# Jackxiini/Tensorflow-distributed-learning

Measured on AMD Instinct MI355X. Metric: images/sec (whole node) MNIST CNN global_batch=64*N, higher is better.
Workload: dtype fp32; 1 GPU; global_batch=64, parallelism=dp1, engine=fused, communicator=local, variant=reference, process_model=single, communicator_impl=LocalCommunicator, ipc_mode=dmabuf, allreduce=local, steps_per_execution=25, graph_captured=True, input_prefetch_executions=1, allreduce_in_graph=False, replicas_identical=True

## Files before the change

csrc/kernels/mnist_cnn.hip:

```cpp
#include <type_traits>

#include "common.h"
#include "mnist_cnn.h"
#include "optim.h"
#include "xgmi_device.h"

namespace tdl {

struct HeadWeights {
  float wa[10], wb[10], b4[10], b3a, b3b;
};

__device__ __forceinline__ HeadWeights load_head_weights(const MnistArgs& a, int l) {
  HeadWeights hw;
  const float* w4 = a.W + a.ow4;
#pragma unroll
  for (int c = 0; c < 10; ++c) {
    hw.wa[c] = w4[l * 10 + c];
    hw.wb[c] = w4[(l + 64) * 10 + c];
    hw.b4[c] = a.W[a.ob4 + c];
  }
  hw.b3a = a.W[a.ob3 + l];
  hw.b3b = a.W[a.ob3 + l + 64];
  return hw;
// ... 426 lines not shown
      const unsigned q = qdc[j];
      const unsigned s = (unsigned)sel[j];
      const f4 v = vdc[j];
      st4(dCs + e4 * 4, f4{(q & 0xffu) == s ? v.x : 0.f, ((q >> 8) & 0xffu) == s ? v.y : 0.f,
                           ((q >> 16) & 0xffu) == s ? v.z : 0.f, (q >> 24) == s ? v.w : 0.f});
    }
  }
#pragma unroll
  for (int j = 0; j < kIp1; ++j) {
    const int e4 = tid + j * 512;
    if (e4 < 169 * 8) st4(P1s + (e4 >> 3) * kP1StrideB + (e4 & 7) * 4, vp1[j]);
  }
#pragma unroll
  for (int j = 0; j < kIwd; ++j) {
    const int e4 = tid + j * 512;
    if (e4 < kLdsWd / 4) st4(Wd + e4 * 4, vwd[j]);
  }
  if (tid < 196) st4(Xs + tid * 4, vx);
  stamp(a.stamps, 1);
  __syncthreads();
  stamp(a.stamps, 2);

  {
    const int t0 = kWgradTiles[half][wave][0], ntiles = kWgradTiles[half][wave][1];
    for (int j = 0; j < ntiles; ++j) {
      const int mt = t0 + j;
      const bool bias_tile = mt == 18;
      const int k = mt * 16 + i;
      const int tap = bias_tile ? 0 : k >> 5, ci = k & 31;
      const int kh = tap / 3, kw = tap - kh * 3;
      const float* pa0 = P1s + (kh * 13 + kw + g) * kP1StrideB + ci;
      const float* paS = pa0 + (g >= 2 ? 3 * kP1StrideB : 0);
      const float* pb0 = dCs + (2 * kDcDim + 2 + g) * kDcStride + 16 * p + i;
      const float* pbS = pb0 + (g >= 2 ? 5 * kDcStride : 0);
      const float unit_a = (i == 0) ? 1.f : 0.f;
      auto kloop = [&](auto bias) {
        f4 c0 = zero4(), c1 = zero4();
#pragma unroll
        for (int s0 = 0; s0 < 25; s0 += 5) {
          float av[5], bv[5];
#pragma unroll
          for (int u = 0; u < 5; ++u) {
            const int st = s0 + u, q = (4 * st) / 10, r = (4 * st) % 10;
            const bool strad = r == 8;
            if constexpr (decltype(bias)::value) av[u] = unit_a;
            else av[u] = (strad ? paS : pa0)[(q * 13 + r) * kP1StrideB];
            bv[u] = (strad ? pbS : pb0)[(q * kDcDim + r) * kDcStride];
          }
#pragma unroll
          for (int u = 0; u < 5; ++u) {
            if ((s0 + u) & 1) c1 = mfma16x16x4(av[u], bv[u], c1);
            else c0 = mfma16x16x4(av[u], bv[u], c0);
          }
        }
        return c0 + c1;
      };
      const f4 acc = bias_tile ? kloop(std::true_type{}) : kloop(std::false_type{});
#pragma unroll
      for (int r = 0; r < 4; ++r) {
        const int row = mt * 16 + 4 * g + r;
        if (row < kMnistPart2Rows) a.part2[((size_t)bi * kMnistPart2Rows + row) * 64 + 16 * p + i] = acc[r];
      }
    }
  }

  stamp(a.stamps, 3);
  float dw[10];
#pragma unroll
  for (int j = 0; j < 10; ++j) dw[j] = 0.f;
  const int d = 7 - wave;
  const int pix0 = half ? kDgSplit : 0, pix1 = half ? 169 : kDgSplit;
  if (d < (pix1 - pix0 + 15) / 16) {
    const int P = pix0 + d * 16 + i;
    const bool valid = P < pix1;
    const int Pc = valid ? P : pix0;
    const int ih = Pc / 13, iw = Pc - ih * 13;
    const float* wb = Wd + (g * 16 + i) * 4;
    const int c = 16 * h + i;
    unsigned q1v[4];
#pragma unroll
    for (int r = 0; r < 4; ++r) {
      const int Pr = min(pix0 + d * 16 + 4 * g + r, pix1 - 1);
      q1v[r] = a.A1[((size_t)bi * 169 + Pr) * 32 + c];
    }
    const int ih_lo = (pix0 + d * 16) / 13, ih_hi = min(pix0 + d * 16 + 15, pix1 - 1) / 13;
    const int kh_lo = max(0, ih_lo - 9), kh_hi = min(2, ih_hi);
    f4 acc0 = zero4(), acc1 = zero4();
    for (int kh = kh_lo; kh <= kh_hi; ++kh) {
#pragma unroll
      for (int kw = 0; kw < 3; ++kw) {
        const int tap = kh * 3 + kw;
        const float* ap = dCs + ((ih - kh + 2) * kDcDim + (iw - kw + 2)) * kDcStride + 4 * g;
#pragma unroll
        for (int c0 = 0; c0 < 64; c0 += 16) {
          const f4 av = ld4(ap + c0);
          const f4 bv = ld4(wb + (tap * 16 + c0 / 4) * 64);
          acc0 = mfma16x16x4(av.x, bv.x, acc0);
          acc1 = mfma16x16x4(av.y, bv.y, acc1);
          acc0 = mfma16x16x4(av.z, bv.z, acc0);
          acc1 = mfma16x16x4(av.w, bv.w, acc1);
        }
      }
    }
    const f4 acc = acc0 + acc1;
    stamp(a.stamps, 6);
#pragma unroll
    for (int r = 0; r < 4; ++r) {
      const int Pr = pix0 + d * 16 + 4 * g + r;
      if (Pr < pix1) {
        const float v = P1s[Pr * kP1StrideB + c] > 0.f ? acc[r] : 0.f;
        const unsigned q1 = q1v[r];
        const int ph = Pr / 13, pw = Pr - ph * 13;
        const float* img = Xs + (2 * ph + (q1 >> 1)) * 28 + 2 * pw + (q1 & 1);
#pragma unroll
        for (int kh = 0; kh < 3; ++kh)
#pragma unroll
          for (int kw = 0; kw < 3; ++kw) dw[kh * 3 + kw] = fmaf(img[kh * 28 + kw], v, dw[kh * 3 + kw]);
        dw[9] += v;
      }
    }
  }
#pragma unroll
  for (int j = 0; j < 10; ++j) dw[j] = sum_lane_groups(dw[j]);
  if (g == 0) {
#pragma unroll
    for (int j = 0; j < 10; ++j) red[(wave * 10 + j) * 16 + i] = dw[j];
  }
  stamp(a.stamps, 4);
  __syncthreads();
  stamp(a.stamps, 5);
  if (tid < 160) {
    const int j = tid >> 4, ii = tid & 15;
    float s = 0.f;
#pragma unroll
    for (int w = 2; w < 8; ++w) s += red[(w * 10 + j) * 16 + ii];
    a.part1[((size_t)bi * 2 + half) * kMnistPart1Cols + j * 32 + 16 * h + ii] = s;
  }
}

constexpr int kLdsFwd = 784 + 320 + 169 * kP1Stride + 72 * 16 * 4 + 400 + 169 * 32 / 4 + 400 / 4 + 16 * 128 + 4 + 128 +
                        288 * 16 +
                        kHeadW;
constexpr int kDcF = 15, kDcFStride = 20;
constexpr int kLdsFwdFused = kLdsFwd + kDcF * kDcF * kDcFStride;
constexpr int kP1Live = 12;
constexpr int kConv1Tiles = kP1Live * kP1Live / 4;
__constant__ int kFusedWgradTiles[8][2] = {{0, 2}, {3, 2}, {7, 3}, {12, 3}, {2, 1}, {5, 2}, {10, 2}, {15, 3}};

__device__ __forceinline__ void bwd_stamp(unsigned long long* buf, int k) {
  if (buf != nullptr && (threadIdx.x & 63) == 0)
    buf[(size_t)gridDim.x * 72 + (blockIdx.x * 8 + (threadIdx.x >> 6)) * 4 + k] = __builtin_amdgcn_s_memrealtime();
}

template <int N>
__device__ __forceinline__ void fused_wgrad_tiles(const MnistArgs& a, int bi, int cq, int t0, const float* P1s,
                                                  const float* dCs) {
  const int lane = threadIdx.x & 63, i = lane & 15, g = lane >> 4;
  const float* pa0[N];
#pragma unroll
  for (int u = 0; u < N; ++u) {
    const int k = (t0 + u) * 16 + i;
    const int tap = k >> 5, ci = k & 31;
    const int kh = tap / 3, kw = tap - kh * 3;
    pa0[u] = P1s + (kh * 13 + kw + g) * kP1Stride + ci;
  }
  const int wrapA = g >= 2 ? 3 * kP1Stride : 0, wrapB = g >= 2 ? 5 * kDcFStride : 0;
  const float* pb0 = dCs + (2 * kDcF + 2 + g) * kDcFStride + i;
  f4 acc[N];
#pragma unroll
  for (int u = 0; u < N; ++u) acc[u] = zero4();
  constexpr int kS = 3, kBlocks = (25 + kS - 1) / kS;
  float bv[2][kS], av[2][kS][N];
  auto load = [&](int buf, int blk) {
#pragma unroll
    for (int j = 0; j < kS; ++j) {
      const int st = blk * kS + j;
      if (st >= 25) break;
      const int q = (4 * st) / 10, r = (4 * st) % 10;
      const bool strad = r == 8;
      bv[buf][j] = pb0[(q * kDcF + r) * kDcFStride + (strad ? wrapB : 0)];
#pragma unroll
      for (int u = 0; u < N; ++u) av[buf][j][u] = pa0[u][(q * 13 + r) * kP1Stride + (strad ? wrapA : 0)];
    }
  };
  load(0, 0);
#pragma unroll
  for (int blk = 0; blk < kBlocks; ++blk) {
    if (blk + 1 < kBlocks) load((blk + 1) & 1, blk + 1);
    __builtin_amdgcn_sched_barrier(0);
#pragma unroll
    for (int j = 0; j < kS; ++j) {
      if (blk * kS + j >= 25) break;
#pragma unroll
      for (int u = 0; u < N; ++u) acc[u] = mfma16x16x4(av[blk & 1][j][u], bv[blk & 1][j], acc[u]);
    }
    __builtin_amdgcn_sched_barrier(0);
  }
  const auto rs = buf_rsrc(a.part2 + (size_t)bi * kP2QuadFloats, kP2QuadFloats * 4);
#pragma unroll
  for (int u = 0; u < N; ++u) st4_sc1(rs, ((((t0 + u) * 4 + g) * 64 + 16 * cq + i) * 4) * 4, acc[u]);
}

__device__ __forceinline__ void lds_dgrad_w2(const float* w2d, f4 (&bwd)[9]) {
  const int wave = __builtin_amdgcn_readfirstlane(threadIdx.x >> 6), lane = threadIdx.x & 63;
  const int i = lane & 15, g = lane >> 4, nt = wave >> 2;
#pragma unroll
  for (int tap = 0; tap < 9; ++tap) bwd[tap] = ld4(w2d + (tap * 32 + 16 * nt + i) * 16 + 4 * g);
}

__device__ __forceinline__ void fused_conv_bwd(const MnistArgs& a, int bi, int cq, const float* dp2s,
                                               const uint8_t* a2s, const float* P1s, const uint8_t* a1s,
                                               const float* xs, float* dCs, float* red, const f4 (&bwd)[9]) {
  const int tid = threadIdx.x, wave = __builtin_amdgcn_readfirstlane(tid >> 6), lane = tid & 63;
  const int i = lane & 15, g = lane >> 4;
  bwd_stamp(a.stamps, 0);

  auto wgrad = [&]() {
    const int t0 = kFusedWgradTiles[wave][0], ntiles = kFusedWgradTiles[wave][1];
    if (ntiles == 2) fused_wgrad_tiles<2>(a, bi, cq, t0, P1s, dCs);
    else if (ntiles == 3) fused_wgrad_tiles<3>(a, bi, cq, t0, P1s, dCs);
    else fused_wgrad_tiles<1>(a, bi, cq, t0, P1s, dCs);
  };
  const bool swap = (a.variant & kMnistVariantStagger) && wave >= 4;
  if (!swap) wgrad();
  bwd_stamp(a.stamps, 1);

  float dw[10];
#pragma unroll
  for (int j = 0; j < 10; ++j) dw[j] = 0.f;
  const int nt = wave >> 2, wt = wave & 3;
  auto dgrad = [&](auto ktiles) {
    constexpr int kT = decltype(ktiles)::value;
    const int ci = 16 * nt + i;
    f4 acc[kT][2];
    int ih[kT], iw[kT], khlo[kT], khhi[kT];
#pragma unroll
    for (int u = 0; u < kT; ++u) {
      const int t = wt + 4 * u;
      const int Pc = min(t * 16 + i, 168);
      ih[u] = Pc / 13;
      iw[u] = Pc - ih[u] * 13;
      const int ih_lo = min(t * 16, 168) / 13, ih_hi = min(t * 16 + 15, 168) / 13;
      khlo[u] = t < 11 ? max(0, ih_lo - 9) : 3;
      khhi[u] = min(2, ih_hi);
      acc[u][0] = zero4();
      acc[u][1] = zero4();
    }
    float p1v[kT][4];
    unsigned q1v[kT][4];
#pragma unroll
    for (int u = 0; u < kT; ++u)
#pragma unroll
      for (int r = 0; r < 4; ++r) {
        const int Pr = min((wt + 4 * u) * 16 + 4 * g + r, 168);
        p1v[u][r] = P1s[Pr * kP1Stride + ci];
        q1v[u][r] = a1s[Pr * 32 + ci];
      }
    f4 av[2][kT];
    auto load = [&](int buf, int tap) {
      const int kh = tap / 3, kw = tap - kh * 3;
#pragma unroll
      for (int u = 0; u < kT; ++u)
        av[buf][u] = ld4(dCs + ((ih[u] - kh + 2) * kDcF + (iw[u] - kw + 2)) * kDcFStride + 4 * g);
    };
    load(0, 0);
#pragma unroll
    for (int tap = 0; tap < 9; ++tap) {
      if (tap + 1 < 9) load((tap + 1) & 1, tap + 1);
      __builtin_amdgcn_sched_barrier(0);
      const int kh = tap / 3;
      const f4 bv = bwd[tap];
#pragma unroll
      for (int u = 0; u < kT; ++u) {
        if (kh < khlo[u] || kh > khhi[u]) continue;
        const f4 x = av[tap & 1][u];
        acc[u][0] = mfma16x16x4(x.x, bv.x, acc[u][0]);
        acc[u][1] = mfma16x16x4(x.y, bv.y, acc[u][1]);
        acc[u][0] = mfma16x16x4(x.z, bv.z, acc[u][0]);
        acc[u][1] = mfma16x16x4(x.w, bv.w, acc[u][1]);
      }
      __builtin_amdgcn_sched_barrier(0);
    }
#pragma unroll
    for (int u = 0; u < kT; ++u) {
      const int t = wt + 4 * u;
      if (t >= 11) continue;
      const f4 ac = acc[u][0] + acc[u][1];
#pragma unroll
      for (int r = 0; r < 4; ++r) {
        const int Pr = t * 16 + 4 * g + r;
        if (Pr < 169) {
          const float v = p1v[u][r] > 0.f ? ac[r] : 0.f;
          const unsigned q1 = q1v[u][r];
          const int ph = Pr / 13, pw = Pr - ph * 13;
          const float* img = xs + (2 * ph + (q1 >> 1)) * 28 + 2 * pw + (q1 & 1);
#pragma unroll
          for (int kh = 0; kh < 3; ++kh)
#pragma unroll
            for (int kw = 0; kw < 3; ++kw) dw[kh * 3 + kw] = fmaf(img[kh * 28 + kw], v, dw[kh * 3 + kw]);
          dw[9] += v;
        }
      }
    }
  };
  if (wt < 2) dgrad(std::integral_constant<int, 3>{});
  else dgrad(std::integral_constant<int, 2>{});
  if (swap) wgrad();
  bwd_stamp(a.stamps, 2);
#pragma unroll
  for (int j = 0; j < 10; ++j) dw[j] = sum_lane_groups(dw[j]);
  if (g == 0) {
#pragma unroll
    for (int j = 0; j < 10; ++j) red[(wave * 10 + j) * 16 + i] = dw[j];
  }
  lds_barrier();
  bwd_stamp(a.stamps, 3);
  if (tid < kMnistPart1Cols) {
    const int j = tid >> 5, c = tid & 31, nt = c >> 4, ii = c & 15;
    float sum = 0.f;
#pragma unroll
    for (int w = 0; w < 4; ++w) sum += red[((4 * nt + w) * 10 + j) * 16 + ii];
    a.part1[((size_t)bi * 4 + cq) * kMnistPart1Cols + tid] = sum;
  }
}

__device__ __forceinline__ void store_saved_fwd(const MnistArgs& a, int bi, int cq, const float* P1s,
                                                const uint8_t* a1s, const float* p2s, const uint8_t* a2s,
                                                int t, int nt) {
  for (int e = (a.fused_bwd ? 676 : 0) + t; e < (a.fused_bwd ? 776 : 2 * 338 + 200); e += nt) {
    if (e < 338) {
      const int e4 = cq * 338 + e, pos = e4 >> 3, c4 = (e4 & 7) * 4;
      st4(a.P1 + (size_t)bi * 5408 + e4 * 4, ld4(P1s + pos * kP1Stride + c4));
    } else if (e < 676) {
      const int w = cq * 338 + (e - 338);
      reinterpret_cast<unsigned*>(a.A1 + (size_t)bi * 5408)[w] = reinterpret_cast<const unsigned*>(a1s)[w];
    } else if (e < 776) {
      const int u = e - 676, wo = u >> 2, q = u & 3;
      st4(a.P2 + (size_t)bi * 1600 + wo * 64 + 16 * cq + 4 * q, ld4(p2s + wo * 16 + 4 * q));
    } else {
      const int u = e - 776, wo = u >> 2, q = u & 3;
      *reinterpret_cast<unsigned*>(a.A2 + (size_t)bi * 1600 + wo * 64 + 16 * cq + 4 * q) =
          reinterpret_cast<const unsigned*>(a2s)[wo * 4 + q];
    }
  }
}

__global__ __launch_bounds__(512) void k_fwd_conv(MnistArgs a) {
  extern __shared__ __attribute__((aligned(16))) float sm[];
  float* xs = sm;
  float* w1s = xs + 784;
  float* P1s = w1s + 320;
  float* w2s = P1s + 169 * kP1Stride;
  float* p2s = w2s + 72 * 16 * 4;
  uint8_t* a1s = reinterpret_cast<uint8_t*>(p2s + 400);
  uint8_t* a2s = a1s + 169 * 32;
  float* red = reinterpret_cast<float*>(a2s + 400);
  int* s_last = reinterpret_cast<int*>(red + 16 * 128);
  float* w2d = red + 16 * 128 + 4 + 128;
  float* hws = w2d + 288 * 16;
  float* dCs = hws + kHeadW;
  const int tid = threadIdx.x, wave = tid >> 6, lane = tid & 63;
  const int i = lane & 15, g = lane >> 4;
  int bi = blockIdx.x >> 2, cq = blockIdx.x & 3;
  if ((a.variant & kMnistVariantXcd) && (a.b & 7) == 0) {
    const int x = blockIdx.x & 7, sl = blockIdx.x >> 3;
    bi = x * (a.b >> 3) + (sl >> 2);
    cq = sl & 3;
  }
  if ((a.variant & kMnistVariantPrio) && __builtin_amdgcn_readfirstlane(wave) >= 4) __builtin_amdgcn_s_setprio(1);
  stamp(a.stamps, 0);
  const int sample = a.idx[bi];
  const f4 vx = ld4(a.X + (size_t)sample * 784 + min(tid, 195) * 4);
  const int label = a.Y[sample];
  const float vw1 = tid < 288 ? a.W[a.ow1 + tid] : a.W[a.ob1 + min(tid - 288, 31)];
  f4 vw2[3];
#pragma unroll
  for (int j = 0; j < 3; ++j) {
    const int e = min(tid + j * 512, 1151);
    vw2[j] = ld4(a.W + a.ow2 + (e >> 2) * 64 + 16 * cq + (e & 3) * 4);
  }
  const float b2v = a.W[a.ob2 + 16 * cq + (lane & 15)];
  const uint32_t tag = a.ep[0] + 1u;
  __builtin_amdgcn_sched_barrier(0);
  if (tid < 196) st4(xs + tid * 4, vx);
  if (tid < 320) w1s[tid] = vw1;
#pragma unroll
  for (int j = 0; j < 3; ++j) {
    const int e = tid + j * 512;
    if (e < 1152) {
      const int k = e >> 2, q = e & 3;
      float* d = w2s + ((k >> 2) * 16 + 4 * q) * 4 + (k & 3);
      d[0] = vw2[j].x;
      d[4] = vw2[j].y;
      d[8] = vw2[j].z;
      d[12] = vw2[j].w;
      st4(w2d + k * 16 + 4 * q, vw2[j]);
    }
  }
  stamp(a.stamps, 1);
  __syncthreads();
  stamp(a.stamps, 2);
  const int n4 = (tid & 31) * 4, rg = tid >> 5;
  f4 w3v[25];
  const auto w3r = buf_rsrc(a.W + a.ow3 + (size_t)16 * cq * 128, (unsigned)((1600 - 16 * cq) * 128 * 4));
  const int w3vo = (rg * 128 + n4) * 4;
  auto ldw3 = [&](int j) { w3v[j] = ld4_buf(w3r, w3vo, j * 64 * 128 * 4); };
#pragma unroll
  for (int j = 0; j < 6; ++j) ldw3(j);
  {
    float bw[2][3];
#pragma unroll
    for (int nt = 0; nt < 2; ++nt)
#pragma unroll
      for (int s3 = 0; s3 < 3; ++s3) {
        const int k = 4 * s3 + g;
        bw[nt][s3] = k < 9 ? w1s[k * 32 + nt * 16 + i] : 0.f;
      }
    int tap_off[3];
#pragma unroll
    for (int s3 = 0; s3 < 3; ++s3) {
      const int k = min(4 * s3 + g, 8);
      tap_off[s3] = (k / 3) * 28 + (k % 3);
    }
    const float bias[2] = {w1s[288 + i], w1s[288 + 16 + i]};
    const int cwave = __builtin_amdgcn_readfirstlane(wave);
    static_assert(kConv1Tiles == 4 * 6 + 4 * 3, "slot -> tile map of conv1");
    auto live = [&](int it, int u) { return cwave < 4 || 2 * it + u < 3; };
    const int mtb = wave < 4 ? wave : 20 + wave;
    float xa[2][2][3];
    auto load_x = [&](int buf, int it) {
      const int mt0 = mtb + 8 * it;
#pragma unroll
      for (int u = 0; u < 2; ++u) {
        if (!live(it, u)) continue;
        const int w = (mt0 + 4 * u) * 4 + (i >> 2), q = i & 3;
        const int ph = w / kP1Live;
        const int y = 2 * ph + (q >> 1), x = 2 * (w - ph * kP1Live) + (q & 1);
        const float* xb = xs + y * 28 + x;
#pragma unroll
        for (int s3 = 0; s3 < 3; ++s3) xa[buf][u][s3] = xb[tap_off[s3]];
      }
    };
    load_x(0, 0);
#pragma unroll
    for (int it = 0; it < 3; ++it) {
      const int mt0 = mtb + 8 * it;
      f4 acc[2][2];
#pragma unroll
      for (int u = 0; u < 2; ++u)
#pragma unroll
        for (int nt = 0; nt < 2; ++nt) acc[u][nt] = zero4();
#pragma unroll
      for (int s3 = 0; s3 < 3; ++s3)
#pragma unroll
        for (int u = 0; u < 2; ++u) {
          if (!live(it, u)) continue;
#pragma unroll
          for (int nt = 0; nt < 2; ++nt) acc[u][nt] = mfma16x16x4(xa[it & 1][u][s3], bw[nt][s3], acc[u][nt]);
        }
// ... 4 lines not shown
#pragma unroll
        for (int j = 6 + 5 * it; j < 11 + 5 * it; ++j) ldw3(j);
        __builtin_amdgcn_sched_barrier(0);
      }
#pragma unroll
      for (int u = 0; u < 2; ++u) {
        if (!live(it, u)) continue;
        const int w = (mt0 + 4 * u) * 4 + g;
        const int ph = w / kP1Live;
        const int wo = ph * 13 + (w - ph * kP1Live);
#pragma unroll
        for (int nt = 0; nt < 2; ++nt) {
          const f4 ac = acc[u][nt];
          float m = ac.x;
          unsigned am = 0;
          if (ac.y > m) { m = ac.y; am = 1; }
          if (ac.z > m) { m = ac.z; am = 2; }
          if (ac.w > m) { m = ac.w; am = 3; }
          const int co = nt * 16 + i;
          const float v = fmaxf(m + bias[nt], 0.f);
          P1s[wo * kP1Stride + co] = v;
          a1s[wo * 32 + co] = (uint8_t)am;
        }
      }
    }
    if (cwave >= 4) {
      const int e = tid - 256;
      if (e < 25 * 8) {
        const int c = e >> 3, c4 = e & 7;
        const int cell = c < 13 ? 12 * 13 + c : (c - 13) * 13 + 12;
        st4(P1s + cell * kP1Stride + 4 * c4, zero4());
        reinterpret_cast<unsigned*>(a1s)[cell * 8 + c4] = 0u;
      }
    }
  }
  stamp(a.stamps, 3);
  lds_barrier();
  stamp(a.stamps, 4);
  if (wave < 7) {
    const int wi = wave * 4 + (i >> 2), q = i & 3;
    const bool valid = wi < 25;
    const int wic = valid ? wi : 0;
    const int ph = wic / 5, pw = wic - ph * 5;
    const int oh = 2 * ph + (q >> 1), ow = 2 * pw + (q & 1);
    const float* ab = P1s + (oh * 13 + ow) * kP1Stride + 4 * g;
    const float* bb = w2s + (g * 16 + i) * 4;
    f4 acc0 = zero4(), acc1 = zero4();
#pragma unroll
    for (int kk = 0; kk < 9; ++kk) {
      const int kh = kk / 3, kw = kk % 3;
#pragma unroll
      for (int cb = 0; cb < 32; cb += 16) {
        const f4 av = ld4(ab + (kh * 13 + kw) * kP1Stride + cb);
        const f4 bv = ld4(bb + ((kk * 32 + cb) / 4) * 64);
        acc0 = mfma16x16x4(av.x, bv.x, acc0);
        acc1 = mfma16x16x4(av.y, bv.y, acc1);
        acc0 = mfma16x16x4(av.z, bv.z, acc0);
        acc1 = mfma16x16x4(av.w, bv.w, acc1);
      }
      __builtin_amdgcn_sched_barrier(0);
      ldw3(16 + kk);
      __builtin_amdgcn_sched_barrier(0);
    }
    const f4 acc = acc0 + acc1;
    stamp(a.stamps, 5);
    const int wo = wave * 4 + g;
    if (wo < 25) {
      float m = acc.x;
      unsigned am = 0;
      if (acc.y > m) { m = acc.y; am = 1; }
      if (acc.z > m) { m = acc.z; am = 2; }
      if (acc.w > m) { m = acc.w; am = 3; }
      const float v = fmaxf(m + b2v, 0.f);
      p2s[wo * 16 + i] = v;
      a2s[wo * 16 + i] = (uint8_t)am;
    }
  } else {
#pragma unroll
    for (int j = 16; j < 25; ++j) ldw3(j);
    if (a.head != 0) {
      float hv[23];
#pragma unroll
      for (int u = 0; u < 23; ++u) {
        const int e = min(lane + 64 * u, 1417);
        hv[u] = a.W[e < 1280 ? a.ow4 + e : (e < 1408 ? a.ob3 + (e - 1280) : a.ob4 + (e - 1408))];
      }
#pragma unroll
      for (int u = 0; u < 23; ++u)
        if (lane + 64 * u < 1418) hws[lane + 64 * u] = hv[u];
    }
    if (a.head == 1 && a.dp2_fwd && a.fused_bwd) {
      for (int e4 = lane; e4 < kDcF * kDcF * kDcFStride / 4; e4 += 64) st4(dCs + e4 * 4, zero4());
    }
  }
  __syncthreads();
  {
    f4 hs = zero4();
#pragma unroll
    for (int j = 0; j < 25; ++j) hs += p2s[j * 16 + rg] * w3v[j];
    st4(red + rg * 128 + n4, hs);
  }
  lds_barrier();
  const bool tagged = a.head == 1 && a.dp2_fwd;
  float* sown = red + 16 * 128 + 4;
  if (tid < 32) {
    f4 hsum = zero4();
#pragma unroll
    for (int k = 0; k < 16; ++k) hsum += ld4(red + k * 128 + 4 * tid);
    if (!tagged) {
      st4_sc1(buf_rsrc(a.part3 + ((size_t)cq * a.b + bi) * 128, 512), tid * 16, hsum);
    } else {
      st4(sown + 4 * tid, hsum);
      unsigned long long* p = a.part3t + ((size_t)cq * a.b + bi) * 128 + 4 * tid;
      const unsigned long long tg = (unsigned long long)tag << 32;
      __hip_atomic_store(p, (unsigned long long)__float_as_uint(hsum.x) | tg, __ATOMIC_RELAXED, __HIP_MEMORY_SCOPE_AGENT);
      __hip_atomic_store(p + 1, (unsigned long long)__float_as_uint(hsum.y) | tg, __ATOMIC_RELAXED,
                         __HIP_MEMORY_SCOPE_AGENT);
      __hip_atomic_store(p + 2, (unsigned long long)__float_as_uint(hsum.z) | tg, __ATOMIC_RELAXED,
                         __HIP_MEMORY_SCOPE_AGENT);
      __hip_atomic_store(p + 3, (unsigned long long)__float_as_uint(hsum.w) | tg, __ATOMIC_RELAXED,
                         __HIP_MEMORY_SCOPE_AGENT);
    }
  }
  stamp(a.stamps, 6);
  if (a.head == 0) {
    store_saved_fwd(a, bi, cq, P1s, a1s, p2s, a2s, tid, 512);
    return;
  }
  HeadWeights hw;
  const int uwave = __builtin_amdgcn_readfirstlane(wave);
  if (uwave == 0) hw = lds_head_weights(hws, lane);
  f4 bwd[9];
  if (a.head == 1 && a.dp2_fwd && a.fused_bwd) lds_dgrad_w2(w2d, bwd);

  if (!tagged) {
    asm volatile("s_waitcnt vmcnt(0)" ::: "memory");
    __syncthreads();
    if (tid == 0) {
      const unsigned old = __hip_atomic_fetch_add(a.cnt + bi, 1u, __ATOMIC_RELAXED, __HIP_MEMORY_SCOPE_AGENT);
      s_last[0] = (old & 3u) == 3u;
    }
  }
  lds_barrier();
  const bool last = tagged || s_last[0] != 0;
  float* sdh = red;
  if (last && uwave == 0) {
    if (a.head == 1) head_row(a, bi, lane, label, hw, sdh, tag, tagged ? sown : nullptr, cq, !tagged || cq == kHeadQuarter);
    else head_eval(a, bi, lane, label, hw);
  }
  if (a.head != 1) return;
  if (!last) store_saved_fwd(a, bi, cq, P1s, a1s, p2s, a2s, tid, 512);
  else if (wave != 0) store_saved_fwd(a, bi, cq, P1s, a1s, p2s, a2s, tid - 64, 448);
  if (!a.dp2_fwd) return;
  lds_barrier();
  if (a.fused_bwd) stamp(a.stamps, 7);
  const f4 dh = ld4(sdh + n4);
  float v[25];
  {
    typedef float f2 __attribute__((ext_vector_type(2)));
    const f2 dlo = {dh.x, dh.y}, dhi = {dh.z, dh.w};
#pragma unroll
    for (int j = 0; j < 25; ++j) {
      f2 t = f2{w3v[j].x, w3v[j].y} * dlo;
      t = __builtin_elementwise_fma(f2{w3v[j].z, w3v[j].w}, dhi, t);
      v[j] = t.x + t.y;
    }
  }
  const float d = reduce_scatter32<25>(v, lane);
  const int j = lane & 31;
  if (a.fused_bwd) {
    float val = 0.f;
    if (j < 25) {
      const int kk = j * 16 + rg;
      val = p2s[kk] > 0.f ? d : 0.f;
      const unsigned am = a2s[kk];
      const int ph = (j * 13) >> 6, pw = j - 5 * ph;
      const int y = 2 * ph + (int)(am >> 1), x = 2 * pw + (int)(am & 1u);
      dCs[((y + 2) * kDcF + x + 2) * kDcFStride + rg] = val;
    }
    float sb = rs_swap16(val, val);
    sb += dpp_xor8(sb);
    sb += dpp_mirror8(sb);
    sb += dpp_xor2(sb);
    sb += dpp_xor1(sb);
    if (j == 0) {
      const auto rs = buf_rsrc(a.part2 + (size_t)bi * kP2QuadFloats, kP2QuadFloats * 4);
      st4_sc1(rs, (((kP2Quads - 1) * 64 + 16 * cq + rg) * 4) * 4, f4{sb, 0.f, 0.f, 0.f});
    }
    lds_barrier();
    fused_conv_bwd(a, bi, cq, p2s, a2s, P1s, a1s, xs, dCs, red, bwd);
    return;
  }
  if (j < 25) {
    const int kk = j * 16 + rg;
    a.dP2[(size_t)bi * 1600 + j * 64 + 16 * cq + rg] = p2s[kk] > 0.f ? d : 0.f;
  }
  stamp(a.stamps, 7);
}

__global__ __launch_bounds__(256) void k_finalize(MnistArgs a, int apply_sgd, int ndb, int nbs, int nb2, int nb1) {
  const float lr = *a.lr;
  int blk = blockIdx.x;
  if (blk < ndb) {
    const int T = blk * 4 + (threadIdx.x >> 6);
    if (T < kDenseTasks) dense_w_task(a, T, threadIdx.x & 63, apply_sgd != 0, lr);
    return;
  }
  blk -= ndb;
  if (blk < nbs) {
    const int e = a.ow3 + blk * 256 + threadIdx.x;
    if (e < a.nslab) a.W[e] -= lr * a.G[e];
    return;
  }
  if (blk < nbs + nb2) {
    const int t = (blk - nbs) * 256 + threadIdx.x;
    const int o = t >> 2, sub = t & 3;
    const int n = kMnistPart2Rows * 64;
    float s = 0.f;
    const int oc = min(o, n - 1);
    const int e = (oc >> 6) < 288 ? a.ow2 + oc : a.ob2 + (oc & 63);
    const float wold = apply_sgd ? a.W[e] : 0.f;
    for (int base = 0; base < a.b; base += 64) {
      float v[16];
#pragma unroll
      for (int j = 0; j < 16; ++j) v[j] = a.part2[(size_t)min(base + sub + 4 * j, a.b - 1) * n + oc];
#pragma unroll
      for (int j = 0; j < 16; ++j) s += (base + sub + 4 * j < a.b) ? v[j] : 0.f;
    }
    s += __shfl_xor(s, 1, 64);
    s += __shfl_xor(s, 2, 64);
    if (sub == 0 && o < n) {
      a.G[e] = s;
      if (apply_sgd) a.W[e] = wold - lr * s;
    }
    return;
  }
  const int t = (blk - nbs - nb2) * 256 + threadIdx.x;
  const int o = t >> 4, sub = t & 15;
  const int rows = mnist_part1_rows(a.b, a.fused_bwd != 0);
  float s = 0.f;
  const int oc = min(o, kMnistPart1Cols - 1);
  const int e = oc < 288 ? a.ow1 + oc : a.ob1 + (oc - 288);
  const float wold = apply_sgd ? a.W[e] : 0.f;
  for (int base = 0; base < rows; base += 128) {
    float v[8];
#pragma unroll
    for (int j = 0; j < 8; ++j) v[j] = a.part1[(size_t)min(base + sub + 16 * j, rows - 1) * kMnistPart1Cols + oc];
#pragma unroll
    for (int j = 0; j < 8; ++j) s += (base + sub + 16 * j < rows) ? v[j] : 0.f;
  }
#pragma unroll
  for (int m = 1; m < 16; m <<= 1) s += __shfl_xor(s, m, 64);
  if (sub == 0 && o < kMnistPart1Cols) {
    a.G[e] = s;
    if (apply_sgd) a.W[e] = wold - lr * s;
  }
}

__device__ __forceinline__ void fx_range(const MnistArgs& a, int j, int& lo, int& cnt, int& nseg, int& stride) {
  nseg = 1;
  stride = 0;
  if (j < kFxW3) {
    lo = a.ow3 + (j >> 1) * 2048 + (j & 1) * 64;
    cnt = 64;
    nseg = 16;
    stride = 128;
  } else if (j < kFxW3 + 4) {
    lo = a.ob3 + 32 * (j - kFxW3);
    cnt = 32;
  } else if (j < kFxW3 + 8) {
    lo = a.ow4 + 320 * (j - kFxW3 - 4);
    cnt = 320;
  } else if (j == kFxW3 + 8) {
    lo = a.ob4;
    cnt = 10;
  } else if (j < kFxDense + kFxConv2) {
    const int qd = (j - kFxDense) >> 1, h = (j - kFxDense) & 1;
    if (qd == kP2Quads - 1) {
      lo = a.ob2 + 32 * h;
      cnt = 32;
    } else {
      lo = a.ow2 + qd * 256 + 32 * h;
      cnt = 32;
      nseg = 4;
      stride = 64;
    }
  } else {
    const int q = j - kFxDense - kFxConv2;
    lo = q < 18 ? a.ow1 + q * 16 : a.ob1 + (q - 18) * 16;
    cnt = 16;
  }
}

template <int R>
__device__ __forceinline__ void finalize_x_body(const MnistArgs& a, int apply_sgd, int j);

template <int R, bool LOOP>
__global__ __launch_bounds__(512) void k_finalize_x(MnistArgs a, int apply_sgd) {
  unsigned long long* sb = a.stamps == nullptr ? nullptr
      : a.stamps + (size_t)a.b * 4 * 104 + ((size_t)blockIdx.x * 8 + (threadIdx.x >> 6)) * 2;
  if (sb != nullptr && (threadIdx.x & 63) == 0) sb[0] = __builtin_amdgcn_s_memrealtime();
  if constexpr (LOOP) {
    for (int j = blockIdx.x; j < kFxBlocks; j += gridDim.x) {
      finalize_x_body<R>(a, apply_sgd, j);
      __syncthreads();
    }
  } else {
    finalize_x_body<R>(a, apply_sgd, blockIdx.x);
  }
  if (sb != nullptr && (threadIdx.x & 63) == 0) sb[1] = __builtin_amdgcn_s_memrealtime();
}

template <int R>
__device__ __forceinline__ void finalize_x_body(const MnistArgs& a, int apply_sgd, int j) {
  const int tid = threadIdx.x, wave = tid >> 6, lane = tid & 63;
  const float lr = *a.lr;
  const bool xchg = R > 1 && a.xchg && apply_sgd;
  if (j == 0 && tid == 4 * 64) a.ep[0] += 1u;
  uint32_t e = 0;
  float* xdst = nullptr;
  int64_t half = 0;
  if (xchg) {
    e = __builtin_amdgcn_readfirstlane(a.xa.epoch[j]) + 1u;
    if (xgmi_failed(a.xa.err)) {
      if (tid == 0) a.xa.epoch[j] = e;
      return;
    }
    half = (int64_t)(e & 1u) * 2 * a.xa.cap;
    xdst = a.xa.p.buf[a.xa.rank] + half;
  }
  const bool sgd_local = R == 1 && apply_sgd;
  const bool keep_g = !((sgd_local || xchg) && (a.variant & kMnistVariantNoG));
  if (j < kFxW3) {
    if (wave < 4) dense_w_task(a, (j >> 1) * 8 + (j & 1) * 4 + wave, lane, sgd_local, lr, xdst, keep_g);
  } else if (j < kFxDense) {
    const int jj = j - kFxW3, t = 2 * jj + wave;
    if (jj < 8 ? wave < 2 : wave == 0)
      dense_w_task(a, jj < 8 ? (t < 8 ? kD1TasksW3 - 8 + t : kD1TasksW3 + t - 8) : kD1TasksW3 + 8, lane, sgd_local, lr,
                   xdst, keep_g);
  } else if (j < kFxDense + kFxConv2) {
    __shared__ f4 fx_red2[8][32];
    const int qd = (j - kFxDense) >> 1, h = (j - kFxDense) & 1, c = tid & 31, grp = tid >> 5;
    const bool biasq = qd == kP2Quads - 1;
// ... 241 lines not shown
```

Measured before the change: 2.765 million images/sec.

## Software-pipeline fused conv dgrad epilogue with MFMA and hoist address precompute

Restructures the fused conv backward dgrad: each tile's ReLU-masked weight-gradient FMAs for the previous tile are interleaved with the next tile's MFMAs using sched_group_barriers. Tap counts per tile are specialised at compile time, so tiles outside the valid kernel rows do no work. Address offsets, P1 values and the first wgrad operand block are precomputed before the barrier, off the critical path. The cost is more register pressure and more complex scheduling.

```diff
diff --git a/csrc/kernels/mnist_cnn.hip b/csrc/kernels/mnist_cnn.hip
--- a/csrc/kernels/mnist_cnn.hip
+++ b/csrc/kernels/mnist_cnn.hip
@@ -602,24 +602,72 @@
     buf[(size_t)gridDim.x * 72 + (blockIdx.x * 8 + (threadIdx.x >> 6)) * 4 + k] = __builtin_amdgcn_s_memrealtime();
 }
 
+__device__ __forceinline__ void dgrad_mfma_stamp(unsigned long long* buf) {
+#ifdef TDL_DIAG_DGRAD_STAMP
+  if (buf != nullptr && (threadIdx.x & 63) == 0)
+    buf[(size_t)gridDim.x * 104 + kFxBlocks * 16 + blockIdx.x * 8 + (threadIdx.x >> 6)] = __builtin_amdgcn_s_memrealtime();
+#endif
+}
+
+constexpr int kWgS = 3;
+struct FusedBwdPre {
+  int wga[3], wgb;
+  float wav[kWgS][3];
+  int dga[3], xo[3][4];
+  float p1v[3][4];
+};
+
+__device__ __forceinline__ int wg_wrap_a(int g) { return g >= 2 ? 3 * kP1Stride : 0; }
+
+__device__ __forceinline__ void fused_bwd_pre(FusedBwdPre& pre, const float* P1s, const uint8_t* a1s) {
+  const int wave = __builtin_amdgcn_readfirstlane(threadIdx.x >> 6), lane = threadIdx.x & 63;
+  const int i = lane & 15, g = lane >> 4;
+  const int t0 = kFusedWgradTiles[wave][0];
+#pragma unroll
+  for (int u = 0; u < 3; ++u) {
+    const int k = min(t0 + u, 17) * 16 + i;
+    const int tap = k >> 5, ci = k & 31;
+    const int kh = tap / 3, kw = tap - kh * 3;
+    pre.wga[u] = (kh * 13 + kw + g) * kP1Stride + ci;
+  }
+  pre.wgb = (2 * kDcF + 2 + g) * kDcFStride + i;
+#pragma unroll
+  for (int j = 0; j < kWgS; ++j) {
+    const int q = (4 * j) / 10, r = (4 * j) % 10;
+#pragma unroll
+    for (int u = 0; u < 3; ++u) pre.wav[j][u] = P1s[pre.wga[u] + (q * 13 + r) * kP1Stride + (r == 8 ? wg_wrap_a(g) : 0)];
+  }
+  const int nt = wave >> 2, wt = wave & 3, ci = 16 * nt + i;
+#pragma unroll
+  for (int u = 0; u < 3; ++u) {
+    const int t = wt + 4 * u;
+    const int Pc = min(t * 16 + i, 168);
+    const int ih = Pc / 13, iw = Pc - ih * 13;
+    pre.dga[u] = ((ih + 2) * kDcF + iw + 2) * kDcFStride + 4 * g;
+#pragma unroll
+    for (int r = 0; r < 4; ++r) {
+      const int Pr = min(t * 16 + 4 * g + r, 168);
+      pre.p1v[u][r] = P1s[Pr * kP1Stride + ci];
+      const int q1 = a1s[Pr * 32 + ci];
+      const int ph = Pr / 13, pw = Pr - ph * 13;
+      pre.xo[u][r] = (2 * ph + (q1 >> 1)) * 28 + 2 * pw + (q1 & 1);
+    }
+  }
+}
+
 template <int N>
 __device__ __forceinline__ void fused_wgrad_tiles(const MnistArgs& a, int bi, int cq, int t0, const float* P1s,
-                                                  const float* dCs) {
+                                                  const float* dCs, const FusedBwdPre& pre) {
   const int lane = threadIdx.x & 63, i = lane & 15, g = lane >> 4;
   const float* pa0[N];
 #pragma unroll
-  for (int u = 0; u < N; ++u) {
-    const int k = (t0 + u) * 16 + i;
-    const int tap = k >> 5, ci = k & 31;
-    const int kh = tap / 3, kw = tap - kh * 3;
-    pa0[u] = P1s + (kh * 13 + kw + g) * kP1Stride + ci;
-  }
-  const int wrapA = g >= 2 ? 3 * kP1Stride : 0, wrapB = g >= 2 ? 5 * kDcFStride : 0;
-  const float* pb0 = dCs + (2 * kDcF + 2 + g) * kDcFStride + i;
+  for (int u = 0; u < N; ++u) pa0[u] = P1s + pre.wga[u];
+  const int wrapA = wg_wrap_a(g), wrapB = g >= 2 ? 5 * kDcFStride : 0;
+  const float* pb0 = dCs + pre.wgb;
   f4 acc[N];
 #pragma unroll
   for (int u = 0; u < N; ++u) acc[u] = zero4();
-  constexpr int kS = 3, kBlocks = (25 + kS - 1) / kS;
+  constexpr int kS = kWgS, kBlocks = (25 + kS - 1) / kS;
   float bv[2][kS], av[2][kS][N];
   auto load = [&](int buf, int blk) {
 #pragma unroll
@@ -630,7 +678,8 @@
       const bool strad = r == 8;
       bv[buf][j] = pb0[(q * kDcF + r) * kDcFStride + (strad ? wrapB : 0)];
 #pragma unroll
-      for (int u = 0; u < N; ++u) av[buf][j][u] = pa0[u][(q * 13 + r) * kP1Stride + (strad ? wrapA : 0)];
+      for (int u = 0; u < N; ++u)
+        av[buf][j][u] = blk == 0 ? pre.wav[j][u] : pa0[u][(q * 13 + r) * kP1Stride + (strad ? wrapA : 0)];
     }
   };
   load(0, 0);
@@ -658,18 +707,134 @@
   for (int tap = 0; tap < 9; ++tap) bwd[tap] = ld4(w2d + (tap * 32 + 16 * nt + i) * 16 + 4 * g);
 }
 
+constexpr int dg_kh_lo(int t) { return (16 * t) / 13 > 9 ? (16 * t) / 13 - 9 : 0; }
+constexpr int dg_kh_hi(int t) { return (16 * t + 15) / 13 < 2 ? (16 * t + 15) / 13 : 2; }
+constexpr int dg_taps(int t) { return 3 * (dg_kh_hi(t) - dg_kh_lo(t) + 1); }
+static_assert(dg_taps(2) == 9 && dg_taps(3) == 9 && dg_taps(6) == 9 && dg_taps(7) == 9, "tile class 2");
+static_assert(dg_taps(0) == 6 && dg_taps(4) == 9 && dg_taps(8) == 9 && dg_taps(1) == 9 && dg_taps(5) == 9 &&
+              dg_taps(9) == 3, "tile classes 0 and 1");
+
+#define TDL_SGB(mask, n) __builtin_amdgcn_sched_group_barrier(mask, n, 0)
+
+template <int WTC>
+__device__ __forceinline__ void fused_dgrad(const FusedBwdPre& pre, const float* dCs, const float* xs,
+                                            const f4 (&bwd)[9], float (&dw)[10], unsigned long long* stamps) {
+  constexpr int kT = WTC < 2 ? 3 : 2;
+  auto lda = [&](int u, int tap) {
+    const int kh = tap / 3, kw = tap - kh * 3;
+    return ld4(dCs + pre.dga[u] - (kh * kDcF + kw) * kDcFStride);
+  };
+  auto ldx = [&](int u, int k, int r) { return xs[pre.xo[u][r] + (k / 3) * 28 + k % 3]; };
+  f4 acc0 = zero4(), acc1 = zero4(), pacc0 = zero4(), pacc1 = zero4();
+  float v[4] = {0.f, 0.f, 0.f, 0.f};
+  f4 av[2];
+  float ev[2][12];
+  float el[9][4];
+  av[0] = lda(0, 3 * dg_kh_lo(WTC));
+  auto tile = [&](auto uc, auto sc) {
+    constexpr int u = decltype(uc)::value, t = WTC + 4 * u, up = u > 0 ? u - 1 : 0;
+    constexpr int s0 = decltype(sc)::value;
+    constexpr int tap0 = 3 * dg_kh_lo(t), nA = dg_taps(t);
+    constexpr int cps = u > 0 ? 9 / nA : 0;
+    constexpr int lps = u + 1 == kT ? 9 / nA : 0;
+    static_assert((u == 0 || cps * nA == 9) && (u + 1 < kT || lps * nA == 9), "epilogue split over the taps");
+    acc0 = zero4();
+    acc1 = zero4();
+#pragma unroll
+    for (int j = 0; j < nA; ++j) {
+      const int p = (s0 + j) & 1;
+      if (j + 1 < nA) {
+        av[p ^ 1] = lda(u, tap0 + j + 1);
+#pragma unroll
+        for (int e = 0; e < 4 * cps; ++e) ev[p ^ 1][e] = ldx(up, (j + 1) * cps + (e >> 2), e & 3);
+      } else if constexpr (u + 1 < kT) {
+        constexpr int ncps = 9 / dg_taps(t + 4);
+        av[p ^ 1] = lda(u + 1, 3 * dg_kh_lo(t + 4));
+#pragma unroll
+        for (int e = 0; e < 4 * ncps; ++e) ev[p ^ 1][e] = ldx(u, e >> 2, e & 3);
+      }
+#pragma unroll
+      for (int e = 0; e < 4 * lps; ++e) el[j * lps + (e >> 2)][e & 3] = ldx(u, j * lps + (e >> 2), e & 3);
+      __builtin_amdgcn_sched_barrier(0);
+      const f4 x = av[p], bv = bwd[tap0 + j];
+      auto fmas = [&](int first, int n) {
+#pragma unroll
+        for (int e = first; e < first + n; ++e) {
+          const int k = j * cps + (e >> 2);
+          dw[k] = fmaf(ev[p][e], v[e & 3], dw[k]);
+        }
+      };
+      if (u > 0 && j == 0) {
+        acc0 = mfma16x16x4(x.x, bv.x, acc0);
+        acc1 = mfma16x16x4(x.y, bv.y, acc1);
+        const f4 ac = pacc0 + pacc1;
+#pragma unroll
+        for (int r = 0; r < 4; ++r) {
+          v[r] = pre.p1v[up][r] > 0.f ? ac[r] : 0.f;
+          dw[9] += v[r];
+        }
+        acc0 = mfma16x16x4(x.z, bv.z, acc0);
+        fmas(0, 2 * cps);
+        acc1 = mfma16x16x4(x.w, bv.w, acc1);
+        fmas(2 * cps, 2 * cps);
+        TDL_SGB(0x8, 2);
+        TDL_SGB(0x2, 16);
+        TDL_SGB(0x8, 1);
+        TDL_SGB(0x2, 2 * cps);
+        TDL_SGB(0x8, 1);
+        TDL_SGB(0x2, 2 * cps);
+      } else {
+        acc0 = mfma16x16x4(x.x, bv.x, acc0);
+        fmas(0, cps);
+        acc1 = mfma16x16x4(x.y, bv.y, acc1);
+        fmas(cps, cps);
+        acc0 = mfma16x16x4(x.z, bv.z, acc0);
+        fmas(2 * cps, cps);
+        acc1 = mfma16x16x4(x.w, bv.w, acc1);
+        fmas(3 * cps, cps);
+        if constexpr (cps > 0) {
+#pragma unroll
+          for (int m = 0; m < 4; ++m) {
+            TDL_SGB(0x8, 1);
+            TDL_SGB(0x2, cps);
+          }
+        }
+      }
+      __builtin_amdgcn_sched_barrier(0);
+    }
+    pacc0 = acc0;
+    pacc1 = acc1;
+  };
+  constexpr int n0 = dg_taps(WTC), n1 = dg_taps(WTC + 4);
+  tile(std::integral_constant<int, 0>{}, std::integral_constant<int, 0>{});
+  tile(std::integral_constant<int, 1>{}, std::integral_constant<int, n0>{});
+  if constexpr (kT == 3) tile(std::integral_constant<int, 2>{}, std::integral_constant<int, n0 + n1>{});
+  dgrad_mfma_stamp(stamps);
+  const f4 ac = pacc0 + pacc1;
+#pragma unroll
+  for (int r = 0; r < 4; ++r) {
+    const float vl = pre.p1v[kT - 1][r] > 0.f ? ac[r] : 0.f;
+#pragma unroll
+    for (int k = 0; k < 9; ++k) dw[k] = fmaf(el[k][r], vl, dw[k]);
+    dw[9] += vl;
+  }
+}
+#undef TDL_SGB
+
 __device__ __forceinline__ void fused_conv_bwd(const MnistArgs& a, int bi, int cq, const float* dp2s,
                                                const uint8_t* a2s, const float* P1s, const uint8_t* a1s,
-                                               const float* xs, float* dCs, float* red, const f4 (&bwd)[9]) {
+                                               const float* xs, float* dCs, float* red, const f4 (&bwd)[9],
+                                               FusedBwdPre& pre) {
   const int tid = threadIdx.x, wave = __builtin_amdgcn_readfirstlane(tid >> 6), lane = tid & 63;
   const int i = lane & 15, g = lane >> 4;
   bwd_stamp(a.stamps, 0);
+  if (wave == 0) fused_bwd_pre(pre, P1s, a1s);
 
   auto wgrad = [&]() {
     const int t0 = kFusedWgradTiles[wave][0], ntiles = kFusedWgradTiles[wave][1];
-    if (ntiles == 2) fused_wgrad_tiles<2>(a, bi, cq, t0, P1s, dCs);
-    else if (ntiles == 3) fused_wgrad_tiles<3>(a, bi, cq, t0, P1s, dCs);
-    else fused_wgrad_tiles<1>(a, bi, cq, t0, P1s, dCs);
+    if (ntiles == 2) fused_wgrad_tiles<2>(a, bi, cq, t0, P1s, dCs, pre);
+    else if (ntiles == 3) fused_wgrad_tiles<3>(a, bi, cq, t0, P1s, dCs, pre);
+    else fused_wgrad_tiles<1>(a, bi, cq, t0, P1s, dCs, pre);
   };
   const bool swap = (a.variant & kMnistVariantStagger) && wave >= 4;
   if (!swap) wgrad();
@@ -678,83 +843,10 @@
   float dw[10];
 #pragma unroll
   for (int j = 0; j < 10; ++j) dw[j] = 0.f;
-  const int nt = wave >> 2, wt = wave & 3;
-  auto dgrad = [&](auto ktiles) {
-    constexpr int kT = decltype(ktiles)::value;
-    const int ci = 16 * nt + i;
-    f4 acc[kT][2];
-    int ih[kT], iw[kT], khlo[kT], khhi[kT];
-#pragma unroll
-    for (int u = 0; u < kT; ++u) {
-      const int t = wt + 4 * u;
-      const int Pc = min(t * 16 + i, 168);
-      ih[u] = Pc / 13;
-      iw[u] = Pc - ih[u] * 13;
-      const int ih_lo = min(t * 16, 168) / 13, ih_hi = min(t * 16 + 15, 168) / 13;
-      khlo[u] = t < 11 ? max(0, ih_lo - 9) : 3;
-      khhi[u] = min(2, ih_hi);
-      acc[u][0] = zero4();
-      acc[u][1] = zero4();
-    }
-    float p1v[kT][4];
-    unsigned q1v[kT][4];
-#pragma unroll
-    for (int u = 0; u < kT; ++u)
-#pragma unroll
-      for (int r = 0; r < 4; ++r) {
-        const int Pr = min((wt + 4 * u) * 16 + 4 * g + r, 168);
-        p1v[u][r] = P1s[Pr * kP1Stride + ci];
-        q1v[u][r] = a1s[Pr * 32 + ci];
-      }
-    f4 av[2][kT];
-    auto load = [&](int buf, int tap) {
-      const int kh = tap / 3, kw = tap - kh * 3;
-#pragma unroll
-      for (int u = 0; u < kT; ++u)
-        av[buf][u] = ld4(dCs + ((ih[u] - kh + 2) * kDcF + (iw[u] - kw + 2)) * kDcFStride + 4 * g);
-    };
-    load(0, 0);
-#pragma unroll
-    for (int tap = 0; tap < 9; ++tap) {
-      if (tap + 1 < 9) load((tap + 1) & 1, tap + 1);
-      __builtin_amdgcn_sched_barrier(0);
-      const int kh = tap / 3;
-      const f4 bv = bwd[tap];
-#pragma unroll
-      for (int u = 0; u < kT; ++u) {
-        if (kh < khlo[u] || kh > khhi[u]) continue;
-        const f4 x = av[tap & 1][u];
-        acc[u][0] = mfma16x16x4(x.x, bv.x, acc[u][0]);
-        acc[u][1] = mfma16x16x4(x.y, bv.y, acc[u][1]);
-        acc[u][0] = mfma16x16x4(x.z, bv.z, acc[u][0]);
-        acc[u][1] = mfma16x16x4(x.w, bv.w, acc[u][1]);
-      }
-      __builtin_amdgcn_sched_barrier(0);
-    }
-#pragma unroll
-    for (int u = 0; u < kT; ++u) {
-      const int t = wt + 4 * u;
-      if (t >= 11) continue;
-      const f4 ac = acc[u][0] + acc[u][1];
-#pragma unroll
-      for (int r = 0; r < 4; ++r) {
-        const int Pr = t * 16 + 4 * g + r;
-        if (Pr < 169) {
-          const float v = p1v[u][r] > 0.f ? ac[r] : 0.f;
-          const unsigned q1 = q1v[u][r];
-          const int ph = Pr / 13, pw = Pr - ph * 13;
-          const float* img = xs + (2 * ph + (q1 >> 1)) * 28 + 2 * pw + (q1 & 1);
-#pragma unroll
-          for (int kh = 0; kh < 3; ++kh)
-#pragma unroll
-            for (int kw = 0; kw < 3; ++kw) dw[kh * 3 + kw] = fmaf(img[kh * 28 + kw], v, dw[kh * 3 + kw]);
-          dw[9] += v;
-        }
-      }
-    }
-  };
-  if (wt < 2) dgrad(std::integral_constant<int, 3>{});
-  else dgrad(std::integral_constant<int, 2>{});
+  const int wt = wave & 3;
+  if (wt == 0) fused_dgrad<0>(pre, dCs, xs, bwd, dw, a.stamps);
+  else if (wt == 1) fused_dgrad<1>(pre, dCs, xs, bwd, dw, a.stamps);
+  else fused_dgrad<2>(pre, dCs, xs, bwd, dw, a.stamps);
   if (swap) wgrad();
   bwd_stamp(a.stamps, 2);
 #pragma unroll
@@ -1065,6 +1157,8 @@
   if (!last) store_saved_fwd(a, bi, cq, P1s, a1s, p2s, a2s, tid, 512);
   else if (wave != 0) store_saved_fwd(a, bi, cq, P1s, a1s, p2s, a2s, tid - 64, 448);
   if (!a.dp2_fwd) return;
+  FusedBwdPre pre;
+  if (a.fused_bwd && uwave != 0) fused_bwd_pre(pre, P1s, a1s);
   lds_barrier();
   if (a.fused_bwd) stamp(a.stamps, 7);
   const f4 dh = ld4(sdh + n4);
@@ -1101,7 +1195,7 @@
       st4_sc1(rs, (((kP2Quads - 1) * 64 + 16 * cq + rg) * 4) * 4, f4{sb, 0.f, 0.f, 0.f});
     }
     lds_barrier();
-    fused_conv_bwd(a, bi, cq, p2s, a2s, P1s, a1s, xs, dCs, red, bwd);
+    fused_conv_bwd(a, bi, cq, p2s, a2s, P1s, a1s, xs, dCs, red, bwd, pre);
     return;
   }
   if (j < 25) {
```

Measured after the change: 2.808 million images/sec, median of 6. 1.6% higher.
